# philgzl/brever

Measured on AMD Instinct MI355X. Metric: utterances/sec (4 s @16 kHz) Conv-TasNet train, higher is better.
Workload: dtype bf16

## Files before the change

brever_amd/csrc/convtasnet.hip:

```cpp
#include <hip/hip_runtime.h>
#include <stdio.h>
#include <stdlib.h>
#include <string.h>
#include <algorithm>
#include <string>
#include <vector>

#include "../../include/brever_hip.h"
#include "status.h"
#include "ctn_layout.h"
#include "gemm_rows.cuh"
#include "gemm_wgrad.cuh"
#include "gemm_ws.cuh"
#include "dwpw2_fused.cuh"
#include "gemm_wgrad_full.cuh"
#include "gemm_wgrad_full128.cuh"

constexpr int kWgSplit = 4;
#include "prep.cuh"
#include "tcn_kernels.cuh"
#include "bwd_fused.cuh"
#include "pw1_bwd.cuh"
#include "cln_kernels.cuh"

// ... 49 lines not shown
struct Layout : CtnLayout<BlockOff> {
  int Np, Kfp, Bnp, Hp, Scp;
  long long p_enc, p_dec_f, p_dec_b, p_bott_f, p_bott_b, p_out_f, p_out_b, p_stamp, n_prepared;

  bool fusable() const {
    return !causal && P == 3 && H == 512 && Bn == 128 && Sc == 128 && nb <= 24 ;
  }
  bool fused_fwd() const { return fusable() && fwd_fuse_requested(); }
  bool pw1_rc() const { return !causal && Hp == RC_H && Bnp == RC_N && pw1_rc_requested(); }

  static int limits(const brv_ctn_config* c) {
    return c->kernel_size < 1 || c->kernel_size > 5 ? fail(-2, "kernel_size must be in [1, 5] in the HIP path") : 0;
  }
  int init(const brv_ctn_config* c) {
    if (int r = CtnLayout::init(c, limits)) return r;
    Np = round_up(N, 64); Kfp = round_up(K, 64); Bnp = round_up(Bn, 64);
    Hp = round_up(H, 64); Scp = round_up(Sc, 64);
    long long q = 0;
    auto ptake = [&](long long n) { long long r = q; q += align_up(n, 128); return r; };
    p_enc = ptake((long long)Np*Kfp);
    p_dec_f = ptake((long long)Kfp*Np);
    p_dec_b = ptake((long long)Np*Kfp);
    p_bott_f = ptake((long long)Bnp*Np);
    p_bott_b = ptake((long long)Np*Bnp);
    for (int i = 0; i < nb; ++i) {
      const int rs = (i < nb - 1 ? Bnp : 0) + Scp;
      blk[i].p_c1_f = ptake((long long)Hp*Bnp);
      blk[i].p_c1_b = ptake((long long)Bnp*Hp);
      blk[i].p_rs_f = ptake((long long)rs*Hp);
      blk[i].p_rs_b = ptake((long long)Hp*rs);
      blk[i].p_c1_fp = ptake((long long)Hp*Bnp);
      blk[i].p_rs_fp = ptake((long long)rs*Hp);
      blk[i].p_rs_bp = ptake((long long)Hp*rs);
      blk[i].p_rs_g = ptake((long long)(Bnp + Scp)*Hp);
      blk[i].p_rs_gp = ptake((long long)(Bnp + Scp)*Hp);
      blk[i].p_lazy = ptake(4LL*(Bnp + Scp));
    }
    p_out_f = ptake((long long)S*Np*Scp);
    p_out_b = ptake((long long)Scp*S*Np);
    p_stamp = ptake(128);
    n_prepared = q;
    return 0;
  }
};

struct Workspace {
  long long w, x, z1, z2, skip, m, y, stats, sums, dpre, dw1, gskip, gout, eA, eB,
      e0, dwt, vg, gcopy, total;
  long long gcopy_stride, eB_stride;
  long long wgpart;
  long long h1, h2, wn, ctab, ctab_stride, cfs, cbt, ident, fake_stats, scratch_stats;
  long long vg_stride, vg_bytes;
  long long x_stride, z_stride;
  long long u, u_stride;
  long long stamp;
  long long stats_bytes;
  void init(const Layout& l, long long B, long long T) {
    long long o = 0;
    auto take = [&](long long bytes) { long long r = o; o += align_up(bytes, 256); return r; };
    const long long BT = B*T;
    w = take(BT*l.Np*2);
    x_stride = align_up(BT*l.Bnp*2, 256);
    x = take(x_stride*l.nb);
    z_stride = align_up(BT*l.Hp*2, 256);
    z1 = take(z_stride*l.nb);
    z2 = take(z_stride*l.nb);
    skip = take(BT*l.Scp*4);
    m = take(BT*l.S*l.Np*2);
    y = take(BT*l.S*l.Np*2);
    stats_bytes = (long long)(1 + 2*l.nb)*B*kStatStride*8;
    stats = take(stats_bytes);
    sums = take(stats_bytes);
    dpre = take(BT*l.S*l.Np*2);
    dw1 = take(BT*l.S*l.Np*2);
    gout = take(BT*(l.Bnp + l.Scp)*2);
    gskip = gout + (long long)l.Bnp*2;
    eA = take(BT*l.Hp*2);
    eB_stride = align_up(BT*l.Hp*2, 256);
    eB = take(eB_stride*l.nb);
    gcopy_stride = align_up(BT*l.Bnp*2, 256);
    gcopy = take(gcopy_stride*l.nb);
    e0 = take(BT*l.Np*2);
    dwt = take(BT*l.Np*2);
    vg_stride = align_up(2LL*l.N + (long long)l.nb*l.H*(5 + l.P) + 1 + 2*l.nb + 2LL*l.Hp, 64);
    vg_bytes = vg_stride*kReplicas*4;
    vg = take(vg_bytes);
    wgpart = take((long long)2*kWgSplit*l.nb*W2_G*l.H*4);
    u_stride = align_up(BT*(l.Bnp + l.Scp)*2, 256);
    u = l.fusable() ? take(u_stride*l.nb) : 0;
    stamp = take(256);
    h1 = h2 = wn = ctab = cfs = cbt = ident = fake_stats = scratch_stats = 0; ctab_stride = 0;
    if (l.causal) {
      h1 = take(z_stride*l.nb);
      h2 = take(z_stride*l.nb);
      wn = take(BT*l.Np*2);
      ctab_stride = align_up(BT*2*4, 256);
      ctab = take(ctab_stride*(1 + 2*l.nb));
      cfs = take(BT*2*4);
      cbt = take(BT*2*4);
      const long long cmax = l.Hp > l.Np ? l.Hp : l.Np;
      ident = take((2*cmax + 64)*4);
      fake_stats = take(B*kStatStride*8);
      scratch_stats = take(B*kStatStride*8);
    }
    total = o;
  }
};

struct Views {
  const Layout& l; Workspace ws; char* base; const bf16_t* prep; int B; long long T;
  Views(const Layout& l_, void* workspace, const void* prepared, int B_, long long T_)
      : l(l_), base((char*)workspace), prep((const bf16_t*)prepared), B(B_), T(T_) { ws.init(l, B, T); }
  double BT() const { return (double)B*(double)T; }
  int ldg() const { return l.Bnp + l.Scp; }
  bf16_t* bf(long long off) const { return (bf16_t*)(base + off); }
  float* f32(long long off) const { return (float*)(base + off); }
  double* stat(int i) const { return (double*)(base + ws.stats) + (long long)i*B*kStatStride; }
  double* sum(int i) const { return (double*)(base + ws.sums) + (long long)i*B*kStatStride; }
  bf16_t* w() const { return bf(ws.w); }
  bf16_t* x(int i) const { return bf(ws.x + ws.x_stride*i); }
  bf16_t* z1(int i) const { return bf(ws.z1 + ws.z_stride*i); }
  bf16_t* z2(int i) const { return bf(ws.z2 + ws.z_stride*i); }
  bf16_t* u(int i) const { return bf(ws.u + ws.u_stride*i); }
  float* skip() const { return f32(ws.skip); }
  bf16_t* m() const { return bf(ws.m); }
  bf16_t* y() const { return bf(ws.y); }
  bf16_t* dpre() const { return bf(ws.dpre); }
  bf16_t* dw1() const { return bf(ws.dw1); }
  bf16_t* gskip() const { return bf(ws.gskip); }
  bf16_t* gout() const { return bf(ws.gout); }
  bf16_t* eA() const { return bf(ws.eA); }
  bf16_t* eB(int i) const { return bf(ws.eB + ws.eB_stride*i); }
  bf16_t* gcopy(int i) const { return bf(ws.gcopy + ws.gcopy_stride*i); }
  bf16_t* e0() const { return bf(ws.e0); }
  bf16_t* dwt() const { return bf(ws.dwt); }
  float* vg() const { return f32(ws.vg); }
  float* vslot(int i) const { return vg() + 2LL*l.N + (long long)l.H*(5 + l.P)*i; }
  float* vslope() const { return vslot(l.nb); }
  float* vscratch() const { return vslope() + 1 + 2*l.nb; }
  bf16_t* wn() const { return bf(ws.wn); }
  bf16_t* h1(int i) const { return bf(ws.h1 + ws.z_stride*i); }
  bf16_t* h2(int i) const { return bf(ws.h2 + ws.z_stride*i); }
  long long cmax() const { return l.Hp > l.Np ? l.Hp : l.Np; }
  float* ones() const { return f32(ws.ident); }
  float* zeros() const { return ones() + cmax(); }
  float* one() const { return zeros() + cmax(); }
  double* fake_stats() const { return (double*)(base + ws.fake_stats); }
  double* scratch_stats() const { return (double*)(base + ws.scratch_stats); }
  float* cfs() const { return f32(ws.cfs); }
  float* cbt() const { return f32(ws.cbt); }
  float* tab(int i) const { return f32(ws.ctab + ws.ctab_stride*i); }
};

template <int BN, int AK, int EM>
int launch_gemm_rows_t(const GemmRowsParams& p0, int batch, hipStream_t st) {
  GemmRowsParams p = p0;
  p.n_ttiles = ceil_div(p.T, GR_BM); p.n_ntiles = ceil_div(p.Np, BN); p.batch = batch;
  dim3 grid(p.n_ttiles*p.n_ntiles*batch);
  hipLaunchKernelGGL((gemm_rows_kernel<BN, AK, EM>), grid, dim3(256), 0, st, p);
  BRV_HIP_OK(hipGetLastError());
  return 0;
}

#ifdef BRV_DIAG
__global__ void diag_stamp_kernel(long long* out, int slot) {
  const long long t = stamp_realtime();
  if (threadIdx.x == 0) {
    out[slot] = t;
    if (slot == 0) { out[2] = 0x7fffffffffffffffLL; out[3] = 0; }
  }
}
long long* debug_buffer() {
  static long long* buf = nullptr;
  if (!buf) {
    if (hipMalloc(&buf, 1 << 20) != hipSuccess) return nullptr;
    (void)hipMemset(buf, 0, 1 << 20);
  }
  return buf;
}
#endif

inline int mode_stamp(bool fused_fwd) { return fused_fwd ? 0x46555345 : 0x504c4149; }
__global__ void stamp_write_kernel(int* dst, int value) { *dst = value; }
__global__ void stamp_check_f64_kernel(const int* stamp, int expect, double* poison, long long n) {
  if (*stamp == expect) return;
  const double nan = __longlong_as_double(0x7ff8000000000000LL);
  for (long long i = threadIdx.x; i < n; i += blockDim.x) poison[i] = nan;
}
struct CallInitParams {
  double* a; long long a_n; void* b; long long b_bytes;
  const int* check; int expect; int* write; int value;
};
__global__ __launch_bounds__(256) void call_init_kernel(const CallInitParams p) {
  const bool bad = *p.check != p.expect;
  const double fill = bad ? __longlong_as_double(0x7ff8000000000000LL) : 0.0;
  const long long tid = (long long)blockIdx.x*256 + threadIdx.x, nth = (long long)gridDim.x*256;
  for (long long i = tid; i < p.a_n; i += nth) p.a[i] = fill;
  if (p.b) {
    unsigned char* b = (unsigned char*)p.b;
    long long head = (16 - ((unsigned long long)b & 15)) & 15;
    if (head > p.b_bytes) head = p.b_bytes;
    const long long n16 = (p.b_bytes - head) >> 4, tail0 = head + (n16 << 4);
    uint4* mid = reinterpret_cast<uint4*>(b + head);
    const uint4 z = make_uint4(0, 0, 0, 0);
    for (long long i = tid; i < n16; i += nth) mid[i] = z;
    for (long long i = tid*4; i < head; i += nth*4) *reinterpret_cast<unsigned int*>(b + i) = 0u;
    for (long long i = tail0 + tid*4; i < p.b_bytes; i += nth*4) *reinterpret_cast<unsigned int*>(b + i) = 0u;
  }
  if (tid == 0 && p.write) *p.write = p.value;
}
inline int launch_call_init(double* a, long long a_n, void* b, long long b_bytes, const int* check, int expect,
                            int* write, int value, hipStream_t st) {
  CallInitParams ip; ip.a = a; ip.a_n = a_n; ip.b = b; ip.b_bytes = b_bytes; ip.check = check; ip.expect = expect;
  ip.write = write; ip.value = value;
  const long long units = a_n + (b_bytes >> 4);
  int gx = (int)std::min<long long>(512, (units + 1023)/1024);
  if (gx < 1) gx = 1;
  hipLaunchKernelGGL(call_init_kernel, dim3(gx), dim3(256), 0, st, ip);
  BRV_HIP_OK(hipGetLastError());
  return 0;
}

int device_cus() {
  static const int n = [] {
    int dev = 0, v = 0;
    if (hipGetDevice(&dev) != hipSuccess ||
        hipDeviceGetAttribute(&v, hipDeviceAttributeMultiprocessorCount, dev) != hipSuccess || v <= 0)
      v = 256;
    return v;
  }();
  return n;
}
int num_cus() {
  const int n = device_cus();
  const int e = t_opts->cu_eighths >= 1 && t_opts->cu_eighths <= 8 ? t_opts->cu_eighths : 8;
  const int m = n*e/8/8*8;
  return m >= 8 ? m : n;
}

template <int KP, int NSL, int WM, int EM, int AT, bool CAT, int NW = 8>
int launch_gemm_ws(const GemmRowsParams& p0, int batch, hipStream_t st) {
  using C = GemmWsCfg<KP, NSL, WM, NW>;
  GemmRowsParams p = p0;
  p.batch = batch;
#ifdef BRV_DIAG
  if (const char* d = getenv("BRV_DBG")) p.dbg = atoi(d);
  if (p.dbg & (64 | 512)) p.dbg_out = debug_buffer();
#endif
  if (!CAT && p.a.K0 <= 0) {
    p.a.p0 = p.a.p1; p.a.ld0 = p.a.ld1; p.a.bs0 = p.a.bs1; p.a.K0 = 1 << 30;
  }
  const int total = ceil_div(p.T, C::BMW)*batch;
  const int groups = p.Np / C::NP;
  int grid = (NW == 8 ? num_cus() : 2*num_cus())/groups;
  if (grid > total) grid = total;
  if (grid < 1) grid = 1;
#ifdef BRV_DIAG
  if (p.dbg & 512) hipLaunchKernelGGL(diag_stamp_kernel, dim3(1), dim3(64), 0, st, debug_buffer() + 131000, 0);
#endif
  hipLaunchKernelGGL((gemm_ws_kernel<KP, NSL, WM, EM, AT, CAT, NW>), dim3(grid, groups),
                     dim3(64*NW), 0, st, p);
#ifdef BRV_DIAG
  if (p.dbg & 512) hipLaunchKernelGGL(diag_stamp_kernel, dim3(1), dim3(64), 0, st, debug_buffer() + 131000, 1);
#endif
  BRV_HIP_OK(hipGetLastError());
  return 0;
}

template <int AK, int EM>
int launch_gemm_rows(const GemmRowsParams& p, int batch, hipStream_t st,
                     const char* label = "gemm_rows", double bytes = 0) {
  if (p.T <= 0 || batch <= 0) return 0;
  ProfScope prof(label, 2.0*batch*p.T*(double)p.Np*p.Kp, bytes, st);
  if (AK == A_BF16 && p.a.nsrc <= 1 && !opt(BRV_OPT_NO_WS)) {
    const bool plain = p.a.slope == nullptr && p.a.stats == nullptr;
    const bool full = p.a.slope != nullptr && p.a.stats != nullptr;
    const bool one_src = p.a.K0 >= p.Kp || p.a.K0 <= 0;
    if ((EM == E_STORE || EM == E_GLN_BWD) && p.Kp == 128 && p.Np == 512 && plain && one_src)
      return launch_gemm_ws<128, 64, 1, (EM == E_STORE ? E_STORE : E_GLN_BWD), 0, false, 8>(p, batch, st);
    if (EM == E_RES_SKIP && p.Kp == 512 && p.Np == 256 && full && one_src)
      return launch_gemm_ws<512, 32, 1, E_RES_SKIP, 1, false>(p, batch, st);
    if (EM == E_GLN_BWD && p.Kp == 256 && p.Np == 512 && plain && one_src)
      return launch_gemm_ws<256, 32, 1, E_GLN_BWD, 0, false, 8>(p, batch, st);
  }
  if (p.Kp % GR_BK != 0 || p.Np % 64 != 0) return fail(-1, "gemm_rows: unpadded dims");
  if (p.Np % 128 == 0) return launch_gemm_rows_t<128, AK, EM>(p, batch, st);
  return launch_gemm_rows_t<64, AK, EM>(p, batch, st);
}

inline int wgrad_target(const char* label, int dflt) {
  (void)label;
  return t_opts->wg_target != 0 ? t_opts->wg_target : dflt;
}

template <int BH, int HK>
int launch_wgrad_t(WgradGroupParams& gp, hipStream_t st, int target) {
  WgradParams& p = gp.base;
  const int nprob = gp.nprob > 0 ? gp.nprob : 1;
  const int tiles = ceil_div(p.Gp, WG_BG)*(p.Hp/BH);
  const int total = p.B*ceil_div(p.T, WG_BT);
  int ns = ceil_div(target > 0 ? target : 384, tiles*nprob);
  if (target < 0) {
    int nb = p.B;
    while (tiles*nprob*nb > 2048 && nb % 2 == 0) nb /= 2;
    if (nb > ns) ns = nb;
  }
  if (ns > total) ns = total;
  if (ns < 1) ns = 1;
  p.nsplit = ns;
  dim3 grid(tiles, ns, nprob);
  hipLaunchKernelGGL((gemm_wgrad_kernel<BH, HK>), grid, dim3(256), 0, st, gp);
  BRV_HIP_OK(hipGetLastError());
  return 0;
}
template <int HK>
int launch_wgrad_group(WgradGroupParams& gp, hipStream_t st, const char* label,
                       double bytes, int target_dflt = 384) {
  const WgradParams& p = gp.base;
  if (p.T <= 0 || p.B <= 0) return 0;
  const int nprob = gp.nprob > 0 ? gp.nprob : 1;
  ProfScope prof(label, 2.0*nprob*p.B*p.T*(double)p.Gp*p.Hp, bytes*nprob, st);
  if (p.Hp % 64 != 0) return fail(-1, "wgrad: unpadded dims");
  const int target = wgrad_target(label, target_dflt);
  if (p.Hp % 128 == 0) return launch_wgrad_t<128, HK>(gp, st, target);
  return launch_wgrad_t<64, HK>(gp, st, target);
}
template <int HK>
int launch_wgrad(WgradParams& p, hipStream_t st, const char* label = "wgrad",
                 double bytes = 0, int target_dflt = 384) {
  WgradGroupParams gp;
  gp.base = p; gp.nprob = 0;
  return launch_wgrad_group<HK>(gp, st, label, bytes, target_dflt);
}

template <template <int> class F, typename... Args>
int dispatch_p(int P, Args&&... args) {
  switch (P) {
    case 1: return F<1>::run(args...);
    case 2: return F<2>::run(args...);
    case 3: return F<3>::run(args...);
    case 4: return F<4>::run(args...);
    case 5: return F<5>::run(args...);
  }
  return fail(-2, "unsupported kernel_size");
}
template <int P> struct DwFwd {
  static int run(const DwParams& p, hipStream_t st) {
    ProfScope prof("dwconv_fwd", 2.0*P*p.B*p.T*(double)p.Cp, 4.0*p.B*p.T*(double)p.Cp, st);
    dim3 grid(ceil_div(p.T, DW_TT_F)*p.B);
    hipLaunchKernelGGL((dwconv_fwd_kernel<P>), grid, dim3(256), 0, st, p);
    BRV_HIP_OK(hipGetLastError());
    return 0;
  }
};
template <int P> struct DwBwd {
  static int run(const DwParams& p, hipStream_t st) {
    if (p.z2in != nullptr) {
      static const char* by_dil[9] = {"dwconv_bwd_d1", "dwconv_bwd_d2", "dwconv_bwd_d4", "dwconv_bwd_d8", "dwconv_bwd_d16",
                                      "dwconv_bwd_d32", "dwconv_bwd_d64", "dwconv_bwd_d128", "dwconv_bwd_dx"};
      int lg = 0; while ((1 << lg) < p.dil && lg < 8) ++lg;
      ProfScope prof(prof_by_dil() ? by_dil[lg] : "dwconv_bwd", 4.0*P*p.B*p.T*(double)p.Cp, 8.0*p.B*p.T*(double)p.Cp, st);
      const int R = hl_rows_per_tooth(p.dil), K = HL_TT/R;
      const int tiles = ceil_div(p.dil, R)*ceil_div((p.T - 1)/p.dil + 1, K);
      dim3 grid(tiles*p.B*(p.Cp/HL_CG));
      const size_t lds = (size_t)hl_window_rows(p.dil, P)*HL_CG*2;
      hipLaunchKernelGGL((dwconv_bwd_halo_kernel<P>), grid, dim3(256), lds, st, p);
      BRV_HIP_OK(hipGetLastError());
      return 0;
    }
    ProfScope prof("dwconv_bwd", 4.0*P*p.B*p.T*(double)p.Cp, 6.0*p.B*p.T*(double)p.Cp, st);
    dim3 grid(ceil_div(p.T, DW_TT_B)*p.B);
    hipLaunchKernelGGL((dwconv_bwd_kernel<P>), grid, dim3(256), 0, st, p);
    BRV_HIP_OK(hipGetLastError());
    return 0;
  }
};

template <int P> struct DwBwdFused {
  static int run(const BwdFusedParams& p0, hipStream_t st) {
    BwdFusedParams p = p0;
    const DwParams& d = p.d;
#ifdef BF_STAMP
    p.dbg = debug_buffer();
#endif
    bf_tile_shape(d.T, d.dil, P, p.K, p.R);
    const int tiles = ceil_div(d.dil, p.R)*ceil_div((d.T - 1)/d.dil + 1, p.K);
    static const char* by_dil[9] = {"dwpw2_bwd_d1", "dwpw2_bwd_d2", "dwpw2_bwd_d4", "dwpw2_bwd_d8", "dwpw2_bwd_d16",
                                    "dwpw2_bwd_d32", "dwpw2_bwd_d64", "dwpw2_bwd_d128", "dwpw2_bwd_dx"};
    int lg = 0; while ((1 << lg) < d.dil && lg < 8) ++lg;
    ProfScope prof(prof_by_dil() ? by_dil[lg] : "dwpw2_bwd", 2.0*d.B*d.T*(double)d.Cp*(p.Kg + 2*P),
                   2.0*d.B*d.T*((double)p.Kg + 3.0*d.Cp), st);
    dim3 grid(ceil_div(tiles*d.B, 8)*8*(d.Cp/HL_CG));
    if (d.C != d.Cp) return fail(-1, "fused backward: channel count must be a multiple of 64");
    if (p.Kg == 256) hipLaunchKernelGGL((dwconv_bwd_fused_kernel<P, 256>), grid, dim3(256), BF_LDS, st, p);
    else if (p.Kg == 128) hipLaunchKernelGGL((dwconv_bwd_fused_kernel<P, 128>), grid, dim3(256), BF_LDS, st, p);
    else return fail(-1, "fused backward: unexpected [res | skip] width");
    BRV_HIP_OK(hipGetLastError());
    return 0;
  }
};

int launch_dz(const DzParams& p, hipStream_t st) {
  ProfScope prof("gln_prelu_bwd", 0, 6.0*p.B*p.T*(double)p.Cp, st);
  const long long per_item = (long long)p.T*(p.Cp/8);
  int gx = (int)((per_item + 256*8 - 1)/(256*8));
  const int cap = 1024/p.B > 1 ? 1024/p.B : 1;
  if (gx > cap) gx = cap;
  if (gx < 1) gx = 1;
  hipLaunchKernelGGL(dz_kernel, dim3(gx, p.B), dim3(256), 0, st, p);
  BRV_HIP_OK(hipGetLastError());
  return 0;
}

ASpec rows_bf16(const void* ptr, int ld, long long T) {
  ASpec a; memset(&a, 0, sizeof(a));
  a.p0 = ptr; a.ld0 = ld; a.bs0 = T*ld; a.K0 = 1 << 30; a.nsrc = 1;
  return a;
}
void set_affine(ASpec& a, const double* stats, const float* g, const float* b, int C,
                long long T) {
  a.stats = stats; a.gamma = g; a.beta = b; a.C = C;
  a.inv_n = 1.0/((double)T*(double)C); a.eps = 1e-8f;
}
ASpec frames_of(const float* wav, long long L, int hop, int K, long long stride = 0) {
  ASpec a; memset(&a, 0, sizeof(a));
  a.p0 = wav; a.hop = hop; a.Kf = K; a.wav_stride = stride > 0 ? stride : L; a.wav_len = (int)L;
  a.K0 = 1 << 30; a.nsrc = 1;
  return a;
}

struct PrepJobC { int src_off, dst_off, scale_off; unsigned short R, C, rows, cols, dst_ld, tr; };
constexpr int kPrepBatch = 168;
struct PrepBatch { PrepJobC jobs[kPrepBatch]; int n; };
static_assert(sizeof(PrepBatch) <= 4096, "kernel argument size");

struct PackJob { long long src_off, dst_off; int N, K, nsl; };
struct PackBatch { PackJob jobs[96]; int n; };
__global__ __launch_bounds__(256) void pack_frag_kernel(bf16_t* prepared, const PackBatch pb) {
  const PackJob j = pb.jobs[blockIdx.y];
  const long long total = (long long)j.N*j.K/8;
  const int KS = j.K/16;
  for (long long i = (long long)blockIdx.x*256 + threadIdx.x; i < total; i += (long long)gridDim.x*256) {
    const int n = (int)(i / (j.K/8)), k = (int)(i % (j.K/8))*8;
    const int slice = n / j.nsl, f = (n % j.nsl)/32, fr = n % 32, s = k/16, fh = (k % 16)/8;
    const long long dst = (long long)slice*j.nsl*j.K + ((long long)(f*KS + s)*64 + fr + 32*fh)*8;
    *reinterpret_cast<uint4*>(prepared + j.dst_off + dst) =
        *reinterpret_cast<const uint4*>(prepared + j.src_off + (long long)n*j.K + k);
  }
}
__global__ __launch_bounds__(256) void prep_weights_kernel(const float* params,
                                                           bf16_t* prepped,
                                                           const PrepBatch pb) {
  const PrepJobC& c = pb.jobs[blockIdx.y];
  PrepJob j;
  j.src_off = c.src_off; j.dst_off = c.dst_off; j.scale_off = c.scale_off;
  j.R = c.R; j.C = c.C; j.rows = c.rows; j.cols = c.cols; j.dst_ld = c.dst_ld; j.tr = c.tr;
  prep_job_run(params, prepped, j, blockIdx.x, gridDim.x);
}

struct LazyPrepBlk { long long res_w, res_b, skip_w, skip_b, beta, wg, out; };
struct LazyPrepParams {
  int nb, H, Hp, Bn, Sc, Bnp, Scp;
  int* stamp; int stamp_value;
  LazyPrepBlk blk[kWgMaxProb];
};
__global__ __launch_bounds__(256) void lazy_prep_kernel(const float* params, bf16_t* prepped,
                                                        const LazyPrepParams p) {
  const LazyPrepBlk& b = p.blk[blockIdx.y];
  float* out = reinterpret_cast<float*>(prepped + b.out);
  const int NP = p.Bnp + p.Scp;
  const int n = blockIdx.x*4 + (threadIdx.x >> 6), lane = threadIdx.x & 63;
  if (blockIdx.x == 0 && blockIdx.y == 0 && threadIdx.x == 0) *p.stamp = p.stamp_value;
  if (n >= NP) return;
  const bool res = n < p.Bnp;
  const int r = res ? n : n - p.Bnp;
  const bool ok = res ? (r < p.Bn && b.res_w >= 0) : r < p.Sc;
  float v0 = 0.f, v1 = 0.f;
  if (ok) {
    const float* W = params + (res ? b.res_w : b.skip_w) + (long long)r*p.H;
    const bf16_t* wg = prepped + b.wg + (long long)n*p.Hp;
    for (int k = lane; k < p.H; k += 64) {
      v0 = __builtin_fmaf(W[k], params[b.beta + k], v0);
      v1 += bf2f(wg[k]);
    }
  }
  for (int o = 32; o; o >>= 1) { v0 += __shfl_xor(v0, o); v1 += __shfl_xor(v1, o); }
  if (lane == 0) {
    out[n] = ok ? v0 + params[(res ? b.res_b : b.skip_b) + r] : 0.f;
    out[NP + n] = v1;
  }
}

struct SkipCombineParams {
  const bf16_t* u; long long u_stride;
  const double* stats; long long stats_stride;
  const bf16_t* prepared; long long lazy_off[kWgMaxProb];
  float* skip; int nb, B, T, Bnp, Scp; double inv_n; float eps;
};
__global__ __launch_bounds__(256) void skip_combine_kernel(const SkipCombineParams p) {
  __shared__ float rs[kWgMaxProb];
  __shared__ float cs[128];
  const int b = blockIdx.y, tid = threadIdx.x;
  const int NP = p.Bnp + p.Scp;
  __shared__ float ms[kWgMaxProb];
  for (int i = tid; i < p.nb; i += 256) {
    const NormStat ns = norm_stat(p.stats + (2 + 2*i)*p.stats_stride, b, p.inv_n, p.eps);
    rs[i] = ns.rstd; ms[i] = ns.mean*ns.rstd;
  }
  __syncthreads();
  for (int n = tid; n < p.Scp; n += 256) {
    float c = 0.f;
    int i = 0;
    for (; i + 8 <= p.nb; i += 8) {
      float a[8], v[8];
#pragma unroll
      for (int k = 0; k < 8; ++k) {
        const float* lz = reinterpret_cast<const float*>(p.prepared + p.lazy_off[i + k]);
        a[k] = lz[p.Bnp + n]; v[k] = lz[NP + p.Bnp + n];
      }
#pragma unroll
      for (int k = 0; k < 8; ++k) c += a[k] - ms[i + k]*v[k];
    }
    for (; i < p.nb; ++i) {
      const float* lz = reinterpret_cast<const float*>(p.prepared + p.lazy_off[i]);
      c += lz[p.Bnp + n] - ms[i]*lz[NP + p.Bnp + n];
    }
    cs[n] = c;
  }
  __syncthreads();
  const int cpr = p.Scp/8;
  const long long per_item = (long long)p.T*cpr;
  for (long long e = (long long)blockIdx.x*256 + tid; e < per_item; e += (long long)gridDim.x*256) {
    const int c0 = (int)(e % cpr)*8; const long long t = e / cpr;
    float acc[8];
#pragma unroll
    for (int j = 0; j < 8; ++j) acc[j] = cs[c0 + j];
    const bf16_t* src = p.u + ((long long)b*p.T + t)*NP + p.Bnp + c0;
    int i = 0;
    for (; i + 8 <= p.nb; i += 8) {
      uint4 q[8];
#pragma unroll
      for (int k = 0; k < 8; ++k) q[k] = *reinterpret_cast<const uint4*>(src + (i + k)*p.u_stride);
#pragma unroll
      for (int k = 0; k < 8; ++k) {
        float f[8];
        unpack8(q[k], f);
        const float r = rs[i + k];
#pragma unroll
        for (int j = 0; j < 8; ++j) acc[j] = __builtin_fmaf(r, f[j], acc[j]);
      }
    }
    for (; i < p.nb; ++i) {
      float f[8];
      unpack8(*reinterpret_cast<const uint4*>(src + i*p.u_stride), f);
      const float r = rs[i];
#pragma unroll
      for (int j = 0; j < 8; ++j) acc[j] = __builtin_fmaf(r, f[j], acc[j]);
    }
    float* dst = p.skip + ((long long)b*p.T + t)*p.Scp + c0;
    *reinterpret_cast<float4*>(dst) = make_float4(acc[0], acc[1], acc[2], acc[3]);
    *reinterpret_cast<float4*>(dst + 4) = make_float4(acc[4], acc[5], acc[6], acc[7]);
  }
}

}

int reduce_vector_grads(const Views& v, float* grads, hipStream_t st, int blk_lo = 0, int blk_hi = 1 << 30,
                        bool do_ln = true, bool do_tcn = true) {
  const Layout& l = v.l;
  const long long vper = (long long)l.H*(5 + l.P);
  {
    VgradParams vp; memset(&vp, 0, sizeof(vp));
    vp.vg = v.vg(); vp.grads = grads; vp.rep_stride = v.ws.vg_stride;
    vp.N = l.N; vp.H = l.H; vp.P = l.P; vp.nb = l.nb;
    vp.ln_g_off = l.ln_g; vp.blk0_off = l.blk[0].conv_w;
    vp.blk_full = l.nb > 1 ? l.blk[1].conv_w - l.blk[0].conv_w : 0;
    const BlockOff& b0 = l.blk[0];
    const BlockOff& bl = l.blk[l.nb - 1];
    vp.o_dconv_w = b0.dconv_w - b0.conv_w; vp.o_dconv_b = b0.dconv_b - b0.conv_w;
    vp.o_n1_g_full = b0.n1_g - b0.conv_w; vp.o_n1_g_last = bl.n1_g - bl.conv_w;
    vp.tcn_prelu_off = l.tcn_prelu;
    vp.blk_lo = blk_lo; vp.blk_hi = blk_hi; vp.do_ln = do_ln; vp.do_tcn = do_tcn;
    if (b0.prelu1 != b0.n1_g + 4LL*l.H || b0.prelu2 != b0.prelu1 + 1)
      return fail(-1, "vgrad_reduce: unexpected PReLU offsets");
    const long long total = 2LL*l.N + vper*l.nb + 1 + 2*l.nb;
    int gx = (int)((total + 255)/256);
    if (gx > 1024) gx = 1024;
    ProfScope prof("vgrad_reduce", 0, 4.0*total*(kReplicas + 2), st);
    hipLaunchKernelGGL(vgrad_reduce_kernel, dim3(gx), dim3(256), 0, st, vp);
    BRV_HIP_OK(hipGetLastError());
  }
  return 0;
}

__global__ void fill_identity_kernel(float* ones, float* zeros, float* one, int n,
                                     double* fake_stats, int B, double sumsq) {
  const int i = blockIdx.x*256 + threadIdx.x;
  if (i < n) { ones[i] = 1.f; zeros[i] = 0.f; }
  if (i == 0) *one = 1.f;
  if (i < B) { fake_stats[stat_sum(i)] = 0.0; fake_stats[stat_sq(i)] = sumsq; }
}

namespace {

int causal_init(const Views& v, hipStream_t st) {
  const Layout& l = v.l;
  const double sumsq = (1.0 - (double)1e-8f)*(double)v.T*(double)l.H;
// ... 1001 lines not shown
```

brever_amd/csrc/gemm_wgrad.cuh:

```cuda
#pragma once
#include "gemm_rows.cuh"
#include "gfx950.cuh"

namespace brv {

struct WgradParams {
  ASpec g;
  ASpec h;
  int B, T;
  int Gp, Hp;
  float* out0; float* out1; int G0p;
  int N0, N1;
  int Kout, ldo;
  float* gbias0; float* gbias1;
  int nsplit;
};

constexpr int kWgMaxProb = 24;
struct WgradProb {
  const void* g0; const void* g1; const void* h;
  float* out0; float* out1; float* gbias0; float* gbias1;
  const float* slope; const double* stats; const float* gamma; const float* beta;
};
struct WgradGroupParams {
  WgradParams base;
  int nprob;
  WgradProb prob[kWgMaxProb];
};

constexpr int WG_BT = 64;
constexpr int WG_BG = 128;

typedef __attribute__((ext_vector_type(8))) short s16x8;

__device__ __forceinline__ bf16x8 tr_frag(const bf16_t* tile, int ld, int row0,
                                          int col0, int lane) {
  const int g4 = lane >> 4, i = lane & 15, q = i >> 2, pp = i & 3;
  const int col = col0 + 16*(g4 & 1) + 4*pp;
  const int row = row0 + 8*(g4 >> 1) + q;
  const bf16_t* p0 = tile + row*ld + col;
#ifndef BRV_WGRAD_SCALAR_FRAG
  const s16x4 lo = lds_read_tr_tracked(p0);
  const s16x4 hi = lds_read_tr_tracked(p0 + 4*ld);
  const s16x8 v = __builtin_shufflevector(lo, hi, 0, 1, 2, 3, 4, 5, 6, 7);
  return __builtin_bit_cast(bf16x8, v);
#else
  const int r = lane & 31, h = lane >> 5;
  s16x8 v;
#pragma unroll
  for (int j = 0; j < 8; ++j) v[j] = (short)tile[(row0 + 8*h + j)*ld + col0 + r];
  return __builtin_bit_cast(bf16x8, v);
#endif
}

template <int BH, int HK>
__global__ __launch_bounds__(256) void gemm_wgrad_kernel(const WgradGroupParams gp) {
  WgradParams p = gp.base;
  int bx = blockIdx.x, by = blockIdx.y, bz = blockIdx.z;
  {
    const int tiles = gridDim.x, pairs = gridDim.y*gridDim.z;
    if ((pairs & 7) == 0) {
      const int L = bx + tiles*(by + (int)gridDim.y*bz);
      const int xcd = L & 7, slot = L >> 3;
      const int pair = (slot / tiles)*8 + xcd;
      bx = slot % tiles; by = pair % (int)gridDim.y; bz = pair / (int)gridDim.y;
    }
  }
  if (gp.nprob > 0) {
    const WgradProb& q = gp.prob[bz];
    p.g.p0 = q.g0; p.g.p1 = q.g1; p.h.p0 = q.h;
    p.out0 = q.out0; p.out1 = q.out1; p.gbias0 = q.gbias0; p.gbias1 = q.gbias1;
    p.h.slope = q.slope; p.h.stats = q.stats; p.h.gamma = q.gamma; p.h.beta = q.beta;
  }
  constexpr int LDG = WG_BG + 32;
  constexpr int LDH = BH + 32;
  constexpr int NT = BH/32;
  constexpr int HCH = BH/32;
  constexpr int HCPR = BH/8;
  __shared__ __attribute__((aligned(16))) bf16_t Gs[WG_BT*LDG];
  __shared__ __attribute__((aligned(16))) bf16_t Hs[WG_BT*LDH];

  const int tid = threadIdx.x, lane = tid & 63, wid = tid >> 6;
  const int n_htiles = p.Hp/BH;
  const int gtile = bx / n_htiles, htile = bx % n_htiles;
  const int n0 = gtile*WG_BG, k0 = htile*BH;
  const int T = p.T;
  const int cpi = ceil_div(T, WG_BT);
  const int total = p.B*cpi;
  const int per = ceil_div(total, p.nsplit);
  const int c_begin = by*per;
  const int c_end = min(total, c_begin + per);

  const int gcc = tid & 15, grow = tid >> 4;
  const int hcc = tid % HCPR, hrow = tid / HCPR;
  constexpr int HRS = 256/HCPR;

  const ASpec& G = p.g;
  const ASpec& H = p.h;
  const int gch = n0 + gcc*8;
  const bool g_first = gch < G.K0;
  const bf16_t* gsrc = reinterpret_cast<const bf16_t*>(g_first ? G.p0 : G.p1);
  const int gld = g_first ? G.ld0 : G.ld1;
  const long long gbs = g_first ? G.bs0 : G.bs1;
  const int gk = g_first ? gch : gch - G.K0;
  const bool g_ok = gch < p.Gp;

  const int hch = k0 + hcc*8;
  const bool h_ok = hch < p.Hp;
  const bool h_aff = H.stats != nullptr;
  const bool h_prelu = H.slope != nullptr;
  const float hslope = h_prelu ? *H.slope : 1.f;
  float hg[8], hb[8];
  load8_masked(h_aff ? H.gamma : nullptr, hch, H.C, hg);
  load8_masked(h_aff ? H.beta : nullptr, hch, H.C, hb);

  uint4 graw[4];
  uint4 hraw_b[HCH];
  float hraw_f[(HK == A_BF16) ? 1 : HCH][8];
  float bias_acc[8];
#pragma unroll
  for (int j = 0; j < 8; ++j) bias_acc[j] = 0.f;

  auto load_chunk = [&](int c) {
    const int b = c / cpi, t0 = (c % cpi)*WG_BT;
#pragma unroll
    for (int ci = 0; ci < 4; ++ci) {
      const int t = t0 + grow + 16*ci;
      graw[ci] = (g_ok && t < T)
          ? *reinterpret_cast<const uint4*>(gsrc + (long long)b*gbs + (long long)t*gld + gk)
          : make_uint4(0, 0, 0, 0);
    }
#pragma unroll
    for (int ci = 0; ci < HCH; ++ci) {
      const int t = t0 + hrow + HRS*ci;
      if (HK == A_BF16) {
        hraw_b[ci] = (h_ok && t < T)
            ? *reinterpret_cast<const uint4*>(reinterpret_cast<const bf16_t*>(H.p0)
                                              + (long long)b*H.bs0 + (long long)t*H.ld0 + hch)
            : make_uint4(0, 0, 0, 0);
      } else if (HK == A_F32) {
        float4 lo = make_float4(0, 0, 0, 0), hi = lo;
        if (h_ok && t < T) {
          const float* s = reinterpret_cast<const float*>(H.p0) + (long long)b*H.bs0 + (long long)t*H.ld0 + hch;
          lo = *reinterpret_cast<const float4*>(s);
          hi = *reinterpret_cast<const float4*>(s + 4);
        }
        float* d = hraw_f[(HK == A_BF16) ? 0 : ci];
        d[0] = lo.x; d[1] = lo.y; d[2] = lo.z; d[3] = lo.w;
        d[4] = hi.x; d[5] = hi.y; d[6] = hi.z; d[7] = hi.w;
      } else {
        const float* wav = reinterpret_cast<const float*>(H.p0) + (long long)b*H.wav_stride;
#pragma unroll
        for (int j = 0; j < 8; ++j) {
          const int k = hch + j;
          const long long idx = (long long)t*H.hop + k;
          float v = 0.f;
          if (t < T && k < H.Kf && idx < H.wav_len) v = wav[idx];
          hraw_f[(HK == A_BF16) ? 0 : ci][j] = v;
        }
      }
    }
  };

  auto store_chunk = [&](int c) {
    const int b = c / cpi, t0 = (c % cpi)*WG_BT;
#pragma unroll
    for (int ci = 0; ci < 4; ++ci) {
      *reinterpret_cast<uint4*>(Gs + (grow + 16*ci)*LDG + gcc*8) = graw[ci];
      if (p.gbias0 || p.gbias1) {
        float f[8]; unpack8(graw[ci], f);
#pragma unroll
        for (int j = 0; j < 8; ++j) bias_acc[j] += f[j];
      }
    }
    NormStat ns = {0.f, 1.f};
    if (h_aff) ns = norm_stat(H.stats, b, H.inv_n, H.eps);
#pragma unroll
    for (int ci = 0; ci < HCH; ++ci) {
      const int row = hrow + HRS*ci;
      uint4 q;
      if (HK == A_BF16 && !h_aff && !h_prelu) {
        q = hraw_b[ci];
      } else {
        float f[8];
        if (HK == A_BF16) unpack8(hraw_b[ci], f);
        else {
#pragma unroll
          for (int j = 0; j < 8; ++j) f[j] = hraw_f[(HK == A_BF16) ? 0 : ci][j];
        }
        if (h_prelu) {
#pragma unroll
          for (int j = 0; j < 8; ++j) f[j] = prelu(f[j], hslope);
        }
        if (h_aff) {
#pragma unroll
          for (int j = 0; j < 8; ++j)
            f[j] = f[j]*(ns.rstd*hg[j]) + (hb[j] - ns.mean*ns.rstd*hg[j]);
        }
        if (t0 + row >= T) {
#pragma unroll
          for (int j = 0; j < 8; ++j) f[j] = 0.f;
        }
        q = pack8(f);
      }
      *reinterpret_cast<uint4*>(Hs + row*LDH + hcc*8) = q;
    }
  };

  f32x16 acc[NT];
#pragma unroll
  for (int j = 0; j < NT; ++j)
#pragma unroll
    for (int i = 0; i < 16; ++i) acc[j][i] = 0.f;

  if (c_begin < c_end) load_chunk(c_begin);
  for (int c = c_begin; c < c_end; ++c) {
    __syncthreads();
    store_chunk(c);
    __syncthreads();
    if (c + 1 < c_end) load_chunk(c + 1);
#pragma unroll
    for (int s = 0; s < WG_BT/16; ++s) {
      const bf16x8 af = tr_frag(Gs, LDG, 16*s, 32*wid, lane);
#pragma unroll
      for (int j = 0; j < NT; ++j) {
        const bf16x8 bfr = tr_frag(Hs, LDH, 16*s, 32*j, lane);
        acc[j] = __builtin_amdgcn_mfma_f32_32x32x16_bf16(af, bfr, acc[j], 0, 0, 0);
      }
    }
  }

  const int fr = lane & 31, fh = lane >> 5;
#pragma unroll
  for (int j = 0; j < NT; ++j) {
    const int k = k0 + 32*j + fr;
#pragma unroll
    for (int i = 0; i < 16; ++i) {
      const int n = n0 + 32*wid + (i & 3) + 8*(i >> 2) + 4*fh;
      if (k < p.Kout) {
        if (n < p.G0p) {
          if (n < p.N0) atomic_add_f32(p.out0 + (long long)n*p.ldo + k, acc[j][i]);
        } else {
          const int n1 = n - p.G0p;
          if (n1 < p.N1) atomic_add_f32(p.out1 + (long long)n1*p.ldo + k, acc[j][i]);
        }
      }
    }
  }
  if ((p.gbias0 || p.gbias1) && htile == 0) {
    __syncthreads();
    float* sc = reinterpret_cast<float*>(Gs);
#pragma unroll
    for (int j = 0; j < 8; ++j) sc[grow*WG_BG + gcc*8 + j] = bias_acc[j];
    __syncthreads();
    if (tid < WG_BG) {
      float s = 0.f;
      for (int r = 0; r < 16; ++r) s += sc[r*WG_BG + tid];
      const int n = n0 + tid;
      if (n < p.G0p) { if (p.gbias0 && n < p.N0) atomic_add_f32(p.gbias0 + n, s); }
      else if (p.gbias1 && n - p.G0p < p.N1) atomic_add_f32(p.gbias1 + (n - p.G0p), s);
    }
  }
}

}
```

Before: 2448.

## Double-buffer wgrad LDS tiles with deeper register prefetch and one barrier per chunk

New measurement: 2454 (median of 4 runs). About the same (+0.2%).

```diff
diff --git a/brever_amd/csrc/convtasnet.hip b/brever_amd/csrc/convtasnet.hip
--- a/brever_amd/csrc/convtasnet.hip
+++ b/brever_amd/csrc/convtasnet.hip
@@ -375,7 +375,7 @@
   int ns = ceil_div(target > 0 ? target : 384, tiles*nprob);
   if (target < 0) {
     int nb = p.B;
-    while (tiles*nprob*nb > 2048 && nb % 2 == 0) nb /= 2;
+    while (tiles*nprob*nb > 768 && nb % 2 == 0) nb /= 2;
     if (nb > ns) ns = nb;
   }
   if (ns > total) ns = total;
diff --git a/brever_amd/csrc/gemm_wgrad.cuh b/brever_amd/csrc/gemm_wgrad.cuh
--- a/brever_amd/csrc/gemm_wgrad.cuh
+++ b/brever_amd/csrc/gemm_wgrad.cuh
@@ -77,8 +77,9 @@
   constexpr int NT = BH/32;
   constexpr int HCH = BH/32;
   constexpr int HCPR = BH/8;
-  __shared__ __attribute__((aligned(16))) bf16_t Gs[WG_BT*LDG];
-  __shared__ __attribute__((aligned(16))) bf16_t Hs[WG_BT*LDH];
+  constexpr bool GLOCAL = BH == 64;
+  __shared__ __attribute__((aligned(16))) bf16_t Gs[(GLOCAL ? 1 : 2)*WG_BT*LDG];
+  __shared__ __attribute__((aligned(16))) bf16_t Hs[2*WG_BT*LDH];
 
   const int tid = threadIdx.x, lane = tid & 63, wid = tid >> 6;
   const int n_htiles = p.Hp/BH;
@@ -90,103 +91,119 @@
   const int per = ceil_div(total, p.nsplit);
   const int c_begin = by*per;
   const int c_end = min(total, c_begin + per);
-
-  const int gcc = tid & 15, grow = tid >> 4;
+  const int nch = c_end - c_begin;
+  if (nch <= 0) return;
+
+  const int gcc = GLOCAL ? lane & 3 : tid & 15, grow = GLOCAL ? lane >> 2 : tid >> 4;
   const int hcc = tid % HCPR, hrow = tid / HCPR;
   constexpr int HRS = 256/HCPR;
 
   const ASpec& G = p.g;
   const ASpec& H = p.h;
-  const int gch = n0 + gcc*8;
-  const bool g_first = gch < G.K0;
+  const int gcol = (GLOCAL ? 32*wid : 0) + gcc*8;
+  const int gch = n0 + gcol;
+  const bool g_ok = gch < p.Gp;
+  const bool g_first = gch < G.K0 || !g_ok;
   const bf16_t* gsrc = reinterpret_cast<const bf16_t*>(g_first ? G.p0 : G.p1);
   const int gld = g_first ? G.ld0 : G.ld1;
   const long long gbs = g_first ? G.bs0 : G.bs1;
   const int gk = g_first ? gch : gch - G.K0;
-  const bool g_ok = gch < p.Gp;
 
   const int hch = k0 + hcc*8;
   const bool h_ok = hch < p.Hp;
-  const bool h_aff = H.stats != nullptr;
-  const bool h_prelu = H.slope != nullptr;
+  const bool h_aff = HK != A_FRAMES && H.stats != nullptr;
+  const bool h_prelu = HK != A_FRAMES && H.slope != nullptr;
   const float hslope = h_prelu ? *H.slope : 1.f;
   float hg[8], hb[8];
   load8_masked(h_aff ? H.gamma : nullptr, hch, H.C, hg);
   load8_masked(h_aff ? H.beta : nullptr, hch, H.C, hb);
 
-  uint4 graw[4];
-  uint4 hraw_b[HCH];
-  float hraw_f[(HK == A_BF16) ? 1 : HCH][8];
+  constexpr int DEPTH = (HK == A_BF16 || (HK == A_F32 && BH == 128)) ? 2 : 1;
+  struct Regs {
+    uint4 g[4];
+    uint4 hb[(HK == A_BF16) ? HCH : 1];
+    float hf[(HK == A_BF16) ? 1 : HCH][8];
+  };
   float bias_acc[8];
 #pragma unroll
   for (int j = 0; j < 8; ++j) bias_acc[j] = 0.f;
 
-  auto load_chunk = [&](int c) {
-    const int b = c / cpi, t0 = (c % cpi)*WG_BT;
+  const int b_begin = c_begin / cpi;
+  const int t_begin = (c_begin - b_begin*cpi)*WG_BT;
+  constexpr int HES = (HK == A_BF16) ? 2 : 4;
+  const long long hbs = (HK == A_FRAMES) ? H.wav_stride : H.bs0;
+  int lt0 = t_begin;
+
+  const int gk_l = g_ok ? gk : 0;
+  const int hch_l = h_ok ? hch : 0;
+  const bf16_t* gl = gsrc + (long long)b_begin*gbs + gk_l;
+  const char* hl = reinterpret_cast<const char*>(H.p0)
+                 + ((long long)b_begin*hbs + (HK == A_FRAMES ? 0 : hch_l))*HES;
+  auto load_chunk = [&](Regs& r) {
 #pragma unroll
     for (int ci = 0; ci < 4; ++ci) {
-      const int t = t0 + grow + 16*ci;
-      graw[ci] = (g_ok && t < T)
-          ? *reinterpret_cast<const uint4*>(gsrc + (long long)b*gbs + (long long)t*gld + gk)
-          : make_uint4(0, 0, 0, 0);
+      const int t = min(lt0 + grow + 16*ci, T - 1);
+      r.g[ci] = *reinterpret_cast<const uint4*>(gl + (long long)t*gld);
     }
 #pragma unroll
     for (int ci = 0; ci < HCH; ++ci) {
-      const int t = t0 + hrow + HRS*ci;
+      const int t = min(lt0 + hrow + HRS*ci, T - 1);
       if (HK == A_BF16) {
-        hraw_b[ci] = (h_ok && t < T)
-            ? *reinterpret_cast<const uint4*>(reinterpret_cast<const bf16_t*>(H.p0)
-                                              + (long long)b*H.bs0 + (long long)t*H.ld0 + hch)
-            : make_uint4(0, 0, 0, 0);
+        r.hb[(HK == A_BF16) ? ci : 0] =
+            *reinterpret_cast<const uint4*>(reinterpret_cast<const bf16_t*>(hl) + (long long)t*H.ld0);
       } else if (HK == A_F32) {
-        float4 lo = make_float4(0, 0, 0, 0), hi = lo;
-        if (h_ok && t < T) {
-          const float* s = reinterpret_cast<const float*>(H.p0) + (long long)b*H.bs0 + (long long)t*H.ld0 + hch;
-          lo = *reinterpret_cast<const float4*>(s);
-          hi = *reinterpret_cast<const float4*>(s + 4);
-        }
-        float* d = hraw_f[(HK == A_BF16) ? 0 : ci];
+        const float* s = reinterpret_cast<const float*>(hl) + (long long)t*H.ld0;
+        const float4 lo = *reinterpret_cast<const float4*>(s);
+        const float4 hi = *reinterpret_cast<const float4*>(s + 4);
+        float* d = r.hf[(HK == A_BF16) ? 0 : ci];
         d[0] = lo.x; d[1] = lo.y; d[2] = lo.z; d[3] = lo.w;
         d[4] = hi.x; d[5] = hi.y; d[6] = hi.z; d[7] = hi.w;
       } else {
-        const float* wav = reinterpret_cast<const float*>(H.p0) + (long long)b*H.wav_stride;
+        const float* wav = reinterpret_cast<const float*>(hl);
+        const int tf = lt0 + hrow + HRS*ci;
 #pragma unroll
         for (int j = 0; j < 8; ++j) {
           const int k = hch + j;
-          const long long idx = (long long)t*H.hop + k;
+          const long long idx = (long long)tf*H.hop + k;
           float v = 0.f;
-          if (t < T && k < H.Kf && idx < H.wav_len) v = wav[idx];
-          hraw_f[(HK == A_BF16) ? 0 : ci][j] = v;
-        }
-      }
-    }
-  };
-
-  auto store_chunk = [&](int c) {
-    const int b = c / cpi, t0 = (c % cpi)*WG_BT;
+          if (tf < T && k < H.Kf && idx < H.wav_len) v = wav[idx];
+          r.hf[(HK == A_BF16) ? 0 : ci][j] = v;
+        }
+      }
+    }
+    lt0 += WG_BT;
+    if (lt0 >= T) { lt0 = 0; gl += gbs; hl += hbs*HES; }
+  };
+
+  int st0 = t_begin, sb = b_begin;
+  NormStat ns = {0.f, 1.f};
+  if (h_aff) ns = norm_stat(H.stats, sb, H.inv_n, H.eps);
+
+  auto store_chunk = [&](const Regs& r, int stage) {
+    bf16_t* Hd = Hs + stage*(WG_BT*LDH);
+    bf16_t* Gd = Gs + (GLOCAL ? 0 : stage*(WG_BT*LDG));
 #pragma unroll
     for (int ci = 0; ci < 4; ++ci) {
-      *reinterpret_cast<uint4*>(Gs + (grow + 16*ci)*LDG + gcc*8) = graw[ci];
+      const uint4 gv = (g_ok && st0 + grow + 16*ci < T) ? r.g[ci] : make_uint4(0, 0, 0, 0);
+      *reinterpret_cast<uint4*>(Gd + (grow + 16*ci)*LDG + gcol) = gv;
       if (p.gbias0 || p.gbias1) {
-        float f[8]; unpack8(graw[ci], f);
+        float f[8]; unpack8(gv, f);
 #pragma unroll
         for (int j = 0; j < 8; ++j) bias_acc[j] += f[j];
       }
     }
-    NormStat ns = {0.f, 1.f};
-    if (h_aff) ns = norm_stat(H.stats, b, H.inv_n, H.eps);
 #pragma unroll
     for (int ci = 0; ci < HCH; ++ci) {
       const int row = hrow + HRS*ci;
       uint4 q;
       if (HK == A_BF16 && !h_aff && !h_prelu) {
-        q = hraw_b[ci];
+        q = (h_ok && st0 + row < T) ? r.hb[(HK == A_BF16) ? ci : 0] : make_uint4(0, 0, 0, 0);
       } else {
         float f[8];
-        if (HK == A_BF16) unpack8(hraw_b[ci], f);
+        if (HK == A_BF16) unpack8(r.hb[(HK == A_BF16) ? ci : 0], f);
         else {
 #pragma unroll
-          for (int j = 0; j < 8; ++j) f[j] = hraw_f[(HK == A_BF16) ? 0 : ci][j];
+          for (int j = 0; j < 8; ++j) f[j] = r.hf[(HK == A_BF16) ? 0 : ci][j];
         }
         if (h_prelu) {
 #pragma unroll
@@ -197,13 +214,18 @@
           for (int j = 0; j < 8; ++j)
             f[j] = f[j]*(ns.rstd*hg[j]) + (hb[j] - ns.mean*ns.rstd*hg[j]);
         }
-        if (t0 + row >= T) {
+        if (!h_ok || st0 + row >= T) {
 #pragma unroll
           for (int j = 0; j < 8; ++j) f[j] = 0.f;
         }
         q = pack8(f);
       }
-      *reinterpret_cast<uint4*>(Hs + row*LDH + hcc*8) = q;
+      *reinterpret_cast<uint4*>(Hd + row*LDH + hcc*8) = q;
+    }
+    st0 += WG_BT;
+    if (st0 >= T) {
+      st0 = 0; ++sb;
+      if (h_aff && sb < p.B) ns = norm_stat(H.stats, sb, H.inv_n, H.eps);
     }
   };
 
@@ -213,21 +235,56 @@
 #pragma unroll
     for (int i = 0; i < 16; ++i) acc[j][i] = 0.f;
 
-  if (c_begin < c_end) load_chunk(c_begin);
-  for (int c = c_begin; c < c_end; ++c) {
-    __syncthreads();
-    store_chunk(c);
-    __syncthreads();
-    if (c + 1 < c_end) load_chunk(c + 1);
+  auto mfma_chunk = [&](int stage) {
+    const bf16_t* Hr = Hs + stage*(WG_BT*LDH);
+    const bf16_t* Gr = Gs + (GLOCAL ? 0 : stage*(WG_BT*LDG));
 #pragma unroll
     for (int s = 0; s < WG_BT/16; ++s) {
-      const bf16x8 af = tr_frag(Gs, LDG, 16*s, 32*wid, lane);
+      const bf16x8 af = tr_frag(Gr, LDG, 16*s, 32*wid, lane);
 #pragma unroll
       for (int j = 0; j < NT; ++j) {
-        const bf16x8 bfr = tr_frag(Hs, LDH, 16*s, 32*j, lane);
+        const bf16x8 bfr = tr_frag(Hr, LDH, 16*s, 32*j, lane);
         acc[j] = __builtin_amdgcn_mfma_f32_32x32x16_bf16(af, bfr, acc[j], 0, 0, 0);
       }
     }
+  };
+  auto full_step = [&](int stage, Regs& r) {
+    mfma_chunk(stage);
+    store_chunk(r, stage ^ 1);
+    load_chunk(r);
+    lds_barrier();
+  };
+  auto tail_step = [&](int i, int stage, Regs& r) {
+    mfma_chunk(stage);
+    if (i + 1 < nch) {
+      store_chunk(r, stage ^ 1);
+      if (i + 1 + DEPTH < nch) load_chunk(r);
+      lds_barrier();
+    }
+  };
+
+  Regs ra, rb;
+  int i = 0;
+  if (nch > 2 + DEPTH) {
+    load_chunk(ra);
+    if (DEPTH == 2) load_chunk(rb);
+    store_chunk(ra, 0);
+    load_chunk(ra);
+    lds_barrier();
+    for (; i + 2 + DEPTH < nch; i += 2) {
+      full_step(0, DEPTH == 2 ? rb : ra);
+      full_step(1, ra);
+    }
+  } else {
+    load_chunk(ra);
+    if (DEPTH == 2 && nch > 1) load_chunk(rb);
+    store_chunk(ra, 0);
+    if (nch > DEPTH) load_chunk(ra);
+    lds_barrier();
+  }
+  for (; i < nch; i += 2) {
+    tail_step(i, 0, DEPTH == 2 ? rb : ra);
+    if (i + 1 < nch) tail_step(i + 1, 1, ra);
   }
 
   const int fr = lane & 31, fh = lane >> 5;
@@ -251,7 +308,7 @@
     __syncthreads();
     float* sc = reinterpret_cast<float*>(Gs);
 #pragma unroll
-    for (int j = 0; j < 8; ++j) sc[grow*WG_BG + gcc*8 + j] = bias_acc[j];
+    for (int j = 0; j < 8; ++j) sc[grow*WG_BG + gcol + j] = bias_acc[j];
     __syncthreads();
     if (tid < WG_BG) {
       float s = 0.f;
```
